# vinayak-gholap1993/Geometric-Multigrid-preconditioners-for-long-range-Coulomb-interaction

Hardware: AMD Instinct MI355X
Metric: DoF/s per CG-iter (GMG-precond Poisson, 3D) (higher is better)
Workload: dtype f64

## Files before the change

### geometric-multigrid-preconditioners-for-long-range-coulomb-interaction_amd/csrc/gmg_coulomb.hip

```cpp
#include "../../include/gmg_coulomb.h"
#include "gmg_device.hpp"
#include "gmg_sgs.hpp"
#include "gmg_sgs_phase.hpp"
#include "gmg_sgs_dep.hpp"
#include "gmg_sgs_reg.hpp"
#ifdef GMG_EXPERIMENTS
#include "gmg_sgs_chain.hpp"
#endif
#include "gmg_lattice.hpp"
#include "gmg_transfer.hpp"
#include <hip/hip_ext.h>

#include <algorithm>
#include <array>
#include <chrono>
#include <cmath>
#include <cstdio>
#include <cstdlib>
#include <cstring>
#include <climits>
#include <map>
#include <string>
#include <thread>
#include <unordered_map>
#include <vector>

#include "gmg_comm.hpp"

using namespace gmg;

namespace {

struct DevCSR {
  int64_t n_rows = 0, n_cols = 0, nnz = 0;
  int32_t *rowptr = nullptr, *col = nullptr;
  double *val = nullptr;
  int32_t *tile_row = nullptr;
  int n_tiles = 0, tiles_per_xcd = 0, grid = 0;
  bool valid = false;
  HaloPlan halo;
  bool sell = false;
  int32_t *slice_ptr = nullptr;
  int32_t *slice_base = nullptr;
  void *sell_vals = nullptr;
  void *sell_cols = nullptr;
  double *sell_dict = nullptr;
  int32_t *sell_spat = nullptr, *sell_pat = nullptr;
// ... 58 lines not shown
  double cheb_lmax = 0.0;
  SgsPlan sgs;
};

}

struct gmg_context {
  int device = 0;
  hipStream_t stream = nullptr;
  int n_levels = 0;
  std::vector<Level> lv;
  DevCSR S;
  double *S_invd = nullptr;
  double *S_tmp = nullptr;
  int smoother = GMG_SMOOTHER_SSOR;
  double omega = 0.5;
  int steps = 2;
  int cheb_degree = 2;
  double cheb_ratio = 30.0, cheb_lmax_user = 0.0;
  double coarse_tol = 1e-10;
  int coarse_maxit = 1000;
  int64_t cg_n = 0;
  double *cg_g = nullptr, *cg_d0 = nullptr, *cg_d1 = nullptr, *cg_h = nullptr;
  double *cg_ring[kXRing] = {};
  int64_t cg_ring_len = 0;
  char *ring_shared[kPeerMaxRanks] = {};
  int64_t ring_stride = 0;
  int64_t peer_meta[kPeerMaxRanks][4 + kPeerMaxRanks] = {};
  unsigned long long peer_tag0 = 1;
  unsigned int *peer_push_cnt = nullptr;
  CGState *st = nullptr;
  CGState *st_host = nullptr;
  CGState st_final{};
  hipEvent_t ev_chunk[2] = {nullptr, nullptr};
  double *part_a = nullptr, *part_b = nullptr;
  double *scal_dev = nullptr;
  double *scal_host = nullptr;
  int *sgs_abort = nullptr;
  int coarse_chunk = 0;
  int sgs_y_slots = 0;
  bool sgs_disable_wave = false, sgs_disable_phase = false, sgs_chain = false, sgs_dep = false, sgs_reg = false, debug_upload = false, sgs_profile = false;
  int sgs_profile_mode = 0;
  int sgs_phase_chunk = 0;
  int sgs_pf_lead_kb = 0;
  bool sgs_phase_nocascade = false;
  bool sgs_phase_nosplit = false;
  int sgs_phase_profile = 0;
  int sgs_groups = 0;
  int sgs_lds_bytes_override = 0;
  bool disable_sell = false, disable_patterns = false, disable_compression = false, disable_sellp = false, disable_rowclass = false, disable_lattice = false;
  int lattice_segments = 0;
  int lattice_max_blocks = 0;
  int sell_grid = 0;
  int sellp_rr = 0;
  double sellp_cost = 4.0;
  int ssor_blocks = 1;
  int ssor_partition = GMG_SSOR_PARTITION_ROWS;
  std::map<int, std::vector<int64_t>> ssor_block_rows;
  int cg_variant = 0;
  int last_coarse_iters = 0;
  int prof_every = 0;
  std::vector<hipEvent_t> ev_a, ev_b;
  std::vector<hipEvent_t> ev_c, ev_d;
  std::vector<hipEvent_t> ev_e, ev_f;
  bool launch_refused = false;
  int ev_used = 0, ev2_used = 0, ev3_used = 0;
  long long sgs_launch_no = 0;
  hipEvent_t timed_start = nullptr, timed_stop = nullptr;
  gmg_stats stats{};
  double *dens_dev = nullptr;
  int64_t dens_cells = 0;
  int dens_nq = 0;
  Comm comm;
  bool dist = false;
  int64_t sys_global = 0, l0_global = 0;
  double *sys_full_a = nullptr, *sys_full_b = nullptr;
  std::string err;
};

namespace {

#define HIPC(call)                                                                                   \
  do {                                                                                               \
    hipError_t e_ = (call);                                                                          \
    if (e_ != hipSuccess) {                                                                          \
      ctx->err = std::string(#call) + ": " + hipGetErrorString(e_);                                  \
      return GMG_ERR_HIP;                                                                            \
    }                                                                                                \
  } while (0)

#define CHK(call)                 \
  do {                            \
// ... 942 lines not shown
        hipLaunchKernelGGL(vec_add_kernel, dim3(g), dim3(kThreads), 0, ctx->stream, u, 1.0, (const double *)y, L.n);
      }
    }
  }
  *u_io = u;
  return launch_status(ctx);
}

void collect_profile_samples(gmg_context *ctx) {
  const int iters = ctx->st_final.iters;
  for (int i = 0; i < ctx->ev_used; ++i) {
    float ms = 0.f;
    if (hipEventElapsedTime(&ms, ctx->ev_a[(size_t)i], ctx->ev_b[(size_t)i]) != hipSuccess) continue;
    if (i * ctx->prof_every < iters) {
      ctx->stats.spmv0_ms_total += ms;
      ctx->stats.spmv0_samples++;
    } else {
      ctx->stats.spmv0_noop_ms_total += ms;
      ctx->stats.spmv0_noop_samples++;
    }
  }
  for (int i = 0; i < ctx->ev2_used; ++i) {
    float ms = 0.f;
    if (hipEventElapsedTime(&ms, ctx->ev_c[(size_t)i], ctx->ev_d[(size_t)i]) != hipSuccess) continue;
    if (i * ctx->prof_every < iters) {
      ctx->stats.cgupd_ms_total += ms;
      ctx->stats.cgupd_samples++;
    }
  }
}

constexpr int64_t kUnfusedMinRowsDecl = 200000;

template <class EnqueueOne>
int run_cg_chunks(gmg_context *ctx, int later_default, EnqueueOne enqueue_one) {
  const int maxit = ctx->coarse_maxit;
  const int last = ctx->last_coarse_iters;
  const int first = ctx->coarse_chunk > 0 ? ctx->coarse_chunk : (last > 8 ? last - (later_default < 6 ? std::max(2, last / 4) : 2) : 16);
  const int later = ctx->coarse_chunk > 0 ? ctx->coarse_chunk : later_default;
  int launched = 0;
  auto launch_chunk = [&](int n, int slot) -> int {
    for (int q = 0; q < n; ++q) {
      const int rc = enqueue_one(launched++);
      if (rc != GMG_OK) return rc;
    }
    CHK(launch_status(ctx));
    HIPC(hipMemcpyAsync(&ctx->st_host[slot], ctx->st, sizeof(CGState), hipMemcpyDeviceToHost, ctx->stream));
    HIPC(hipEventRecord(ctx->ev_chunk[slot], ctx->stream));
    return GMG_OK;
  };
  int slot = 0;
  CHK(launch_chunk(std::min(first, maxit + 1), slot));
  const bool speculate = !l0_partitioned(ctx) || ctx->comm.peer;
  for (;;) {
    if (speculate) CHK(launch_chunk(later, slot ^ 1));
    for (;;) {
      const hipError_t e = hipEventQuery(ctx->ev_chunk[slot]);
      if (e == hipSuccess) break;
      if (e != hipErrorNotReady) { ctx->err = std::string("hipEventQuery: ") + hipGetErrorString(e); return GMG_ERR_HIP; }
    }
    if (ctx->st_host[slot].done) { ctx->st_final = ctx->st_host[slot]; ctx->stats.coarse_enqueued += launched; break; }
    if (launched > maxit + 2 * later + 2) return fail(ctx, GMG_ERR_HIP, "coarse CG state machine did not terminate");
    if (!speculate) CHK(launch_chunk(later, slot ^ 1));
    slot ^= 1;
  }
  return GMG_OK;
}


int coarse_solve_unfused(gmg_context *ctx, double *x, const double *b, int *iters_out, double *res_out);
void collect_profile_samples(gmg_context *ctx);

int coarse_solve(gmg_context *ctx, double *x, const double *b, int *iters_out, double *res_out) {
// ... 954 lines not shown
    tiles.push_back((int32_t)e);
    r = e;
  }
  return tiles;
}

DevCSR *which_matrix(gmg_context *ctx, int which) {
  if (which == GMG_SYSTEM) return &ctx->S;
  if (which < 0 || which >= ctx->n_levels) return nullptr;
  return &ctx->lv[(size_t)which].A;
}

}

#include "gmg_dist.hpp"


extern "C" {

int gmg_create(gmg_context **out, int device_id, int n_levels) {
  if (!out || n_levels < 1) return GMG_ERR_INVALID;
  *out = nullptr;
  int count = 0;
  if (hipGetDeviceCount(&count) != hipSuccess || count <= 0 || device_id < 0 || device_id >= count) return GMG_ERR_HIP;
  if (hipSetDevice(device_id) != hipSuccess) return GMG_ERR_HIP;
  gmg_context *ctx = new gmg_context();
  ctx->device = device_id;
  ctx->n_levels = n_levels;
  ctx->lv.resize((size_t)n_levels);
  auto bail = [&](int code) { gmg_destroy(ctx); return code; };
  if (hipStreamCreateWithFlags(&ctx->stream, hipStreamNonBlocking) != hipSuccess) return bail(GMG_ERR_HIP);
  if (hipMalloc(&ctx->st, sizeof(CGState)) != hipSuccess) return bail(GMG_ERR_HIP);
  if (hipHostMalloc((void **)&ctx->st_host, 2 * sizeof(CGState), hipHostMallocDefault) != hipSuccess) return bail(GMG_ERR_HIP);
  for (auto &e : ctx->ev_chunk)
    if (hipEventCreateWithFlags(&e, hipEventDisableTiming) != hipSuccess) return bail(GMG_ERR_HIP);
  if (hipMalloc(&ctx->part_a, sizeof(double) * 4 * kMaxPartials) != hipSuccess) return bail(GMG_ERR_HIP);
  if (hipMalloc(&ctx->part_b, sizeof(double) * 4 * kMaxPartials) != hipSuccess) return bail(GMG_ERR_HIP);
  if (hipMalloc(&ctx->scal_dev, sizeof(double) * 8) != hipSuccess) return bail(GMG_ERR_HIP);
  if (hipHostMalloc((void **)&ctx->scal_host, sizeof(double) * 8, hipHostMallocDefault) != hipSuccess) return bail(GMG_ERR_HIP);
  if (hipHostMalloc((void **)&ctx->sgs_abort, sizeof(int), hipHostMallocDefault) != hipSuccess) return bail(GMG_ERR_HIP);
  *ctx->sgs_abort = 0;
  (void)hipMemsetAsync(ctx->st, 0, sizeof(CGState), ctx->stream);
  if (const char *env = std::getenv("GMG_OPTIONS")) {
    std::string all(env);
    size_t pos = 0;
    while (pos < all.size()) {
      size_t end = all.find(',', pos);
      if (end == std::string::npos) end = all.size();
      const std::string item = all.substr(pos, end - pos);
      pos = end + 1;
      const size_t eq = item.find('=');
      if (item.empty()) continue;
      const std::string key = eq == std::string::npos ? item : item.substr(0, eq);
      const double v = eq == std::string::npos ? 1.0 : std::atof(item.c_str() + eq + 1);
      if (gmg_set_option(ctx, key.c_str(), v) != GMG_OK) return bail(GMG_ERR_INVALID);
    }
  }
  *out = ctx;
  return GMG_OK;
}

int gmg_destroy(gmg_context *ctx) {
  if (!ctx) return GMG_OK;
  (void)hipSetDevice(ctx->device);
  if (ctx->stream) (void)hipStreamSynchronize(ctx->stream);
  release_operators(ctx);
  if (ctx->peer_push_cnt) (void)hipFree(ctx->peer_push_cnt);
  if (ctx->dens_dev) (void)hipFree(ctx->dens_dev);
  comm_destroy(ctx->comm);
  for (double *p : {ctx->part_a, ctx->part_b, ctx->scal_dev})
    if (p) (void)hipFree(p);
  if (ctx->st) (void)hipFree(ctx->st);
  if (ctx->st_host) (void)hipHostFree(ctx->st_host);
  for (auto &e : ctx->ev_chunk)
    if (e) (void)hipEventDestroy(e);
  if (ctx->scal_host) (void)hipHostFree(ctx->scal_host);
  if (ctx->sgs_abort) (void)hipHostFree(ctx->sgs_abort);
  for (auto *v : {&ctx->ev_a, &ctx->ev_b, &ctx->ev_c, &ctx->ev_d, &ctx->ev_e, &ctx->ev_f})
    for (hipEvent_t e : *v) (void)hipEventDestroy(e);
  if (ctx->stream) (void)hipStreamDestroy(ctx->stream);
  delete ctx;
  return GMG_OK;
}

int gmg_reset(gmg_context *ctx, int n_levels) {
  if (!ctx || n_levels < 1) return GMG_ERR_INVALID;
  (void)hipSetDevice(ctx->device);
  HIPC(hipStreamSynchronize(ctx->stream));
  release_operators(ctx);
  ctx->n_levels = n_levels;
  ctx->lv.assign((size_t)n_levels, Level());
  ctx->last_coarse_iters = 0;
  ctx->stats = gmg_stats{};
  ctx->ev3_used = 0;
  return GMG_OK;
}

const char *gmg_last_error(const gmg_context *ctx) { return ctx ? ctx->err.c_str() : "null context"; }

int gmg_synchronize(gmg_context *ctx) {
  if (!ctx) return GMG_ERR_INVALID;
  HIPC(hipStreamSynchronize(ctx->stream));
  return GMG_OK;
}

int gmg_set_system_matrix(gmg_context *ctx, int64_t n_rows, int64_t n_cols, const int64_t *rowptr, const int32_t *col,
// ... 862 lines not shown
  for (int pass = 0; pass < 2; ++pass) {
    HIPC(hipEventRecord(e0, ctx->stream));
    for (int r = 0; r < reps; ++r)
      hipLaunchKernelGGL(stream_copy_kernel, dim3(kMaxPartials * 2), dim3(kThreads), 0, ctx->stream, (const double2 *)a, b, n2);
    HIPC(hipEventRecord(e1, ctx->stream));
    HIPC(hipEventSynchronize(e1));
    HIPC(hipEventElapsedTime(&ms, e0, e1));
  }
  if (copy_gbps) *copy_gbps = (double)n2 * 32 * reps / (ms * 1e-3) / 1e9;
  (void)hipEventDestroy(e0); (void)hipEventDestroy(e1);
  (void)hipFree(a); (void)hipFree(b);
  return GMG_OK;
}

int gmg_set_option(gmg_context *ctx, const char *key, double value) {
  if (!ctx || !key) return GMG_ERR_INVALID;
  const std::string k(key);
  const bool on = value != 0.0;
  if (k == "host_threads") g_host_threads = (int)value;
  else if (k == "debug_upload") ctx->debug_upload = on;
  else if (k == "disable_sell") ctx->disable_sell = on;
  else if (k == "disable_patterns") ctx->disable_patterns = on;
  else if (k == "disable_compression") ctx->disable_compression = on;
  else if (k == "disable_sellp") ctx->disable_sellp = on;
  else if (k == "disable_rowclass") ctx->disable_rowclass = on;
  else if (k == "disable_lattice") ctx->disable_lattice = on;
  else if (k == "lattice_segments") ctx->lattice_segments = (int)value;
  else if (k == "lattice_max_blocks") ctx->lattice_max_blocks = (int)value;
  else if (k == "sell_grid") ctx->sell_grid = (int)value;
  else if (k == "sellp_cost") ctx->sellp_cost = value;
  else if (k == "sellp_rr") ctx->sellp_rr = (int)value;
  else if (k == "cg_variant") ctx->cg_variant = (int)value;
  else if (k == "coarse_chunk") ctx->coarse_chunk = (int)value;
  else if (k == "ssor_balanced") ctx->ssor_partition = on ? GMG_SSOR_PARTITION_BALANCED : GMG_SSOR_PARTITION_ROWS;
  else if (k == "sgs_y_slots") ctx->sgs_y_slots = (int)value;
  else if (k == "sgs_disable_wave") ctx->sgs_disable_wave = on;
  else if (k == "sgs_disable_phase") ctx->sgs_disable_phase = on;
  else if (k == "sgs_dep") ctx->sgs_dep = on;
  else if (k == "sgs_reg") ctx->sgs_reg = on;
  else if (k == "sgs_pf_lead_kb") ctx->sgs_pf_lead_kb = (int)value;
  else if (k == "sgs_chain") {
#ifndef GMG_EXPERIMENTS
    if (on) return fail(ctx, GMG_ERR_UNSUPPORTED, "sgs_chain needs a -DGMG_EXPERIMENTS build (tools/build_experiments.sh)");
#endif
    ctx->sgs_chain = on;
  }
  else if (k == "sgs_phase_profile") {
    if (on && ctx->dist && ctx->comm.n_ranks > 1) return fail(ctx, GMG_ERR_INVALID, "sgs_phase_profile: one rank only (the instrumented sweep is a single-GPU measurement)");
    ctx->sgs_phase_profile = (int)value;
  }
  else if (k == "sgs_phase_nosplit") ctx->sgs_phase_nosplit = on;
  else if (k == "sgs_phase_nocascade") ctx->sgs_phase_nocascade = on;
  else if (k == "sgs_phase_chunk") ctx->sgs_phase_chunk = (int)value;
  else if (k == "sgs_groups") ctx->sgs_groups = (int)value;
  else if (k == "sgs_lds_bytes_override") ctx->sgs_lds_bytes_override = (int)value;
  else if (k == "sgs_profile") {
    if (on && ctx->dist && ctx->comm.n_ranks > 1) return fail(ctx, GMG_ERR_INVALID, "sgs_profile: one rank only");
    ctx->sgs_profile = on;
    ctx->sgs_profile_mode = (int)value - 1;
#ifndef GMG_EXPERIMENTS
    if (ctx->sgs_profile_mode > 0) return fail(ctx, GMG_ERR_UNSUPPORTED, "sgs_profile modes > 1 need a -DGMG_EXPERIMENTS build (tools/build_experiments.sh)");
#endif
  }
  else return fail(ctx, GMG_ERR_INVALID, "gmg_set_option: unknown key");
  return GMG_OK;
}
// ... 70 lines not shown
```

### geometric-multigrid-preconditioners-for-long-range-coulomb-interaction_amd/csrc/gmg_device.hpp

```cpp
#pragma once
#include <hip/hip_runtime.h>
#include <stdint.h>

#include <type_traits>

namespace gmg {

constexpr int kThreads = 256;
constexpr int kTileNnz = 4096;
constexpr int kPasses = kTileNnz / (kThreads * 4);
constexpr int kMaxPartials = 2048;


__device__ __forceinline__ double wave_sum(double v) {
#pragma unroll
  for (int off = 32; off > 0; off >>= 1) v += __shfl_down(v, off, 64);
  return v;
}

__device__ __forceinline__ double wave_max(double v) {
#pragma unroll
  for (int off = 32; off > 0; off >>= 1) v = fmax(v, __shfl_down(v, off, 64));
  return v;
}

__device__ __forceinline__ double block_sum(double v, double *scratch ) {
  v = wave_sum(v);
  const int lane = threadIdx.x & 63, wid = threadIdx.x >> 6;
  __syncthreads();
  if (lane == 0) scratch[wid] = v;
  __syncthreads();
  return ((scratch[0] + scratch[1]) + scratch[2]) + scratch[3];
}

__device__ __forceinline__ double block_max(double v, double *scratch) {
  v = wave_max(v);
  const int lane = threadIdx.x & 63, wid = threadIdx.x >> 6;
  __syncthreads();
  if (lane == 0) scratch[wid] = v;
  __syncthreads();
  return fmax(fmax(scratch[0], scratch[1]), fmax(scratch[2], scratch[3]));
}

__device__ __forceinline__ double reduce_partials(const double *p, int n, double *scratch) {
  double s = 0.0;
  for (int i = threadIdx.x; i < n; i += kThreads) s += p[i];
  return block_sum(s, scratch);
}


constexpr int kXRing = 8;

struct CGState {
  double gh[2];
  double res0;
  double res;
  int it_k1;
  int it_k2;
  int done;
  int status;
  int iters;
  int pad;
  double alpha[kXRing];
};

constexpr int kPeerRanks = 8;
constexpr int kPeerCgOffset = 4096;
struct PeerCG {
  char *area;
  char *peer_area[kPeerRanks];
  int n_ranks, me;
  unsigned nb_mask;
  unsigned long long tag0;
  int *abort_flag;
};
constexpr long long kPeerCgSpinLimit = 30000000LL;

__device__ __forceinline__ bool peer_cg_wait(const PeerCG &pc, const unsigned long long *tags, unsigned mask, unsigned long long want) {
  __shared__ int ok_s;
  if (threadIdx.x == 0) {
// ... 45 lines not shown
  double *w;
  double omega, c1;
  const double *g;
  double *dnew;
  CGState *st;
  const double *part_in;
  int n_part_in;
  double *part_out;
  double tol;
  int maxit;
};

__device__ __forceinline__ bool cg_open_iteration(CGState *st, const double *part_in, int n_part_in, double tol, int maxit,
                                                  double *red, double *beta_out) {
  if (st->done) return false;
  const double gg = reduce_partials(part_in, n_part_in, red);
  const double res = sqrt(gg);
  const int it = st->it_k2;
  const bool conv = res <= tol;
  const bool fail = !conv && (it >= maxit || res != res);
  const bool writer = blockIdx.x == 0 && threadIdx.x == 0;
  if (conv || fail) {
    if (writer) {
      st->done = 1;
      st->status = conv ? 0 : 1;
      st->res = res;
      st->iters = it;
      if (it == 0) st->res0 = res;
    }
    return false;
  }
  const double gh_new = res * res;
  *beta_out = (it == 0) ? 0.0 : gh_new / st->gh[(it & 1) ^ 1];
  if (writer) {
    st->gh[it & 1] = gh_new;
    st->it_k1 = it;
    if (it == 0) st->res0 = res;
  }
  return true;
}

template <int MODE, int CG>
__global__ __launch_bounds__(kThreads) void spmv_tile_kernel(SpmvArgs a) {
  __shared__ __attribute__((aligned(16))) double prod[kTileNnz + 8];
  __shared__ double red[4];
  const int tid = threadIdx.x;
  constexpr bool XFORM = (CG == 1);

  double beta = 0.0;
  if constexpr (CG == 1) {
    if (!cg_open_iteration(a.st, a.part_in, a.n_part_in, a.tol, a.maxit, red, &beta)) return;
  }
  if constexpr (CG == 2) {
    if (a.st->done) return;
  }

  const int xcd = blockIdx.x & 7, lb = blockIdx.x >> 3, nb = gridDim.x >> 3;
  const int t_begin = xcd * a.tiles_per_xcd;
  const int t_end = min(t_begin + a.tiles_per_xcd, a.n_tiles);
  double dot_acc = 0.0;

  for (int t = t_begin + lb; t < t_end; t += nb) {
    const int r0 = a.tile_row[t], r1 = a.tile_row[t + 1];
    const int k0 = a.rowptr[r0], k1 = a.rowptr[r1];
    const int ka = k0 & ~3;
    if (k1 - ka <= kTileNnz) {
// ... 541 lines not shown
        const uchar4 k0 = kq;
        if (q + 1 < qe) { kq = kbase[(size_t)(q + 1) * 64]; cols_of(q + 1, c); }
        acc += dict[k0.x] * v0; acc += dict[k0.y] * v1; acc += dict[k0.z] * v2; acc += dict[k0.w] * v3;
      }
    }
    if (valid) finish(row, acc, self, have_self);
    ++s;
  }
  if constexpr (CG != 0) {
    const double sblock = block_sum(dot_acc, red);
    if (threadIdx.x == 0) a.part_out[blockIdx.x] = sblock;
  }
}

struct CGDirArgs {
  double *d;
  const double *d_old;
  const double *g;
  int64_t n;
  CGState *st;
  const double *part_in;
  int n_part_in;
  double tol;
  int maxit;
  PeerCG pc;
  int n_nb;
  int nb_rank[kPeerRanks];
  const int32_t *send_idx;
  int send_off[kPeerRanks + 1];
  double *peer_ghost[kPeerRanks];
  long long peer_stride[kPeerRanks];
  unsigned int *cnt;
  int n_push_wg;
};
__global__ __launch_bounds__(kThreads) void cg_direction_kernel(CGDirArgs a) {
  __shared__ double red[4];
  if (a.st->done) return;
  const int64_t n2 = a.n >> 1;
  const double2 *o2 = reinterpret_cast<const double2 *>(a.d_old);
  const double2 *g2 = reinterpret_cast<const double2 *>(a.g);
  double2 *d2 = reinterpret_cast<double2 *>(a.d);
  const int64_t i0 = (int64_t)blockIdx.x * kThreads + threadIdx.x, stride = (int64_t)gridDim.x * kThreads;
  double2 ov{0.0, 0.0}, gv{0.0, 0.0};
  if (i0 < n2) { ov = o2[i0]; gv = g2[i0]; }
  double beta = 0.0;
  const int it = a.st->it_k2;
  if (!cg_open_iteration(a.st, a.part_in, a.n_part_in, a.tol, a.maxit, red, &beta)) return;
  for (int64_t i = i0; i < n2; i += stride) {
    if (i != i0) { ov = o2[i]; gv = g2[i]; }
    double2 dv;
    dv.x = beta * ov.x - gv.x; dv.y = beta * ov.y - gv.y;
    d2[i] = dv;
  }
  if ((a.n & 1) && blockIdx.x == 0 && threadIdx.x == 0) {
    const int64_t i = a.n - 1;
    a.d[i] = beta * a.d_old[i] - a.g[i];
  }
  if (a.pc.area && (int)blockIdx.x < a.n_push_wg) {
    for (int i = 0; i < a.n_nb; ++i) {
      double *dst = a.peer_ghost[i] + (long long)(it & 7) * a.peer_stride[i];
      const int cnt = a.send_off[i + 1] - a.send_off[i];
      for (int k = blockIdx.x * kThreads + threadIdx.x; k < cnt; k += a.n_push_wg * kThreads) {
        const int li = a.send_idx[a.send_off[i] + k];
        dst[k] = beta * a.d_old[li] - a.g[li];
      }
    }
    __threadfence_system();
    __syncthreads();
    if (threadIdx.x == 0 && atomicAdd(a.cnt, 1u) == (unsigned)a.n_push_wg - 1u) {
      *a.cnt = 0;
      for (int i = 0; i < a.n_nb; ++i)
        __hip_atomic_store(reinterpret_cast<unsigned long long *>(a.pc.peer_area[a.nb_rank[i]] + 2048 + (it & 7) * 64) + a.pc.me,
                           a.pc.tag0 + (unsigned long long)it + 1ull, __ATOMIC_RELEASE, __HIP_MEMORY_SCOPE_SYSTEM);
    }
  }
}

struct PeerSumArgs {
  PeerCG pc;
  const double *part;
// ... 84 lines not shown
  if (i0 < n2) { dv = d2[i0]; hv = h2[i0]; xv = x2[i0]; gv = g2[i0]; }
  const double dh = reduce_partials(a.part_dh, a.n_part_dh, red);
  const int it = a.st->it_k1;
  const double alpha = a.st->gh[it & 1] / dh;
  double acc = 0.0;
  for (int64_t i = i0; i < n2; i += stride) {
    if (i != i0) { dv = d2[i]; hv = h2[i]; xv = x2[i]; gv = g2[i]; }
    xv.x += alpha * dv.x; xv.y += alpha * dv.y;
    gv.x += alpha * hv.x; gv.y += alpha * hv.y;
    x2[i] = xv; g2[i] = gv;
    acc += gv.x * gv.x;
    acc += gv.y * gv.y;
  }
  if ((a.n & 1) && blockIdx.x == 0 && threadIdx.x == 0) {
    const int64_t i = a.n - 1;
    a.x[i] += alpha * a.d[i];
    const double gi = a.g[i] + alpha * a.h[i];
    a.g[i] = gi;
    acc += gi * gi;
  }
  const double s = block_sum(acc, red);
  if (threadIdx.x == 0) a.part_gg[blockIdx.x] = s;
  if (blockIdx.x == 0 && threadIdx.x == 0) a.st->it_k2 = it + 1;
}

struct CGUpdateGArgs {
  double *g;
  const double *h;
  int64_t n;
  CGState *st;
  const double *part_dh;
  int n_part_dh;
  double *part_gg;
};
__global__ __launch_bounds__(kThreads) void cg_update_g_kernel(CGUpdateGArgs a) {
  __shared__ double red[4];
  if (a.st->done) return;
  const int64_t n2 = a.n >> 1;
  const double2 *h2 = reinterpret_cast<const double2 *>(a.h);
  double2 *g2 = reinterpret_cast<double2 *>(a.g);
  const int64_t i0 = (int64_t)blockIdx.x * kThreads + threadIdx.x, stride = (int64_t)gridDim.x * kThreads;
  double2 hv{0.0, 0.0}, gv{0.0, 0.0};
  if (i0 < n2) { hv = h2[i0]; gv = g2[i0]; }
  const int it = a.st->it_k1;
  const double dh = reduce_partials(a.part_dh, a.n_part_dh, red);
  const double alpha = a.st->gh[it & 1] / dh;
  double acc = 0.0;
  for (int64_t i = i0; i < n2; i += stride) {
    if (i != i0) { hv = h2[i]; gv = g2[i]; }
    gv.x += alpha * hv.x; gv.y += alpha * hv.y;
    g2[i] = gv;
    acc += gv.x * gv.x;
    acc += gv.y * gv.y;
  }
  if ((a.n & 1) && blockIdx.x == 0 && threadIdx.x == 0) {
    const int64_t i = a.n - 1;
    const double gi = a.g[i] + alpha * a.h[i];
    a.g[i] = gi;
    acc += gi * gi;
  }
  const double s = block_sum(acc, red);
  if (threadIdx.x == 0) a.part_gg[blockIdx.x] = s;
  if (blockIdx.x == 0 && threadIdx.x == 0) {
    a.st->alpha[it % kXRing] = alpha;
    a.st->it_k2 = it + 1;
  }
}

struct CGXFlushArgs {
  double *x;
  const double *ring[kXRing];
  int64_t n;
  const CGState *st;
  int lo, upto;
};
__global__ __launch_bounds__(kThreads) void cg_xflush_kernel(CGXFlushArgs a) {
  const int hi = min(a.st->it_k2, a.upto);
  if (hi <= a.lo) return;
  const int64_t n2 = a.n >> 1;
// ... 295 lines not shown
```

### geometric-multigrid-preconditioners-for-long-range-coulomb-interaction_amd/csrc/gmg_dist.hpp

```cpp
#pragma once

namespace {

constexpr int64_t kUnfusedMinRows = 200000;

int coarse_solve_unfused(gmg_context *ctx, double *x, const double *b, int *iters_out, double *res_out) {
  Level &L0 = ctx->lv[0];
  DevCSR &A = L0.A;
  const bool comm = l0_partitioned(ctx);
  const int64_t n = L0.n;
  const int g_vec = grid_for(n);
  const int g_upd = grid_for(n / 2);
  double *s_gg = ctx->scal_dev + 4, *s_dh = ctx->scal_dev + 5;
  const bool peer = comm && ctx->comm.peer;
  if (!ctx->cg_ring[0]) {
    if (peer) {
      ctx->ring_stride = (A.n_cols + 2 + 15) / 16 * 16;
      if (comm_share_alloc(ctx->comm, sizeof(double) * (size_t)(ctx->ring_stride * kXRing), ctx->ring_shared))
        return fail(ctx, GMG_ERR_COMM, "coarse CG: shared direction vectors could not be mapped");
      for (int r = 0; r < kXRing; ++r) ctx->cg_ring[r] = reinterpret_cast<double *>(ctx->ring_shared[ctx->comm.rank]) + (int64_t)r * ctx->ring_stride;
      int64_t mine[4 + kPeerMaxRanks];
      mine[0] = ctx->ring_stride; mine[1] = n; mine[2] = mine[3] = 0;
      for (int r = 0; r < kPeerMaxRanks; ++r) mine[4 + r] = -1;
      int64_t ro = 0;
      for (int i = 0; i < A.halo.n_neighbors; ++i) { mine[4 + A.halo.rank[(size_t)i]] = ro; ro += A.halo.recv_count[(size_t)i]; }
      if (comm_exchange_meta(ctx->comm, mine, 4 + kPeerMaxRanks, ctx->peer_meta)) return fail(ctx, GMG_ERR_COMM, "coarse CG: meta exchange failed");
      if (!ctx->peer_push_cnt) {
        HIPC(hipMalloc(&ctx->peer_push_cnt, sizeof(unsigned int)));
        HIPC(hipMemsetAsync(ctx->peer_push_cnt, 0, sizeof(unsigned int), ctx->stream));
      }
    } else {
      for (int r = 0; r < kXRing; ++r) CHK(alloc_vec(ctx, &ctx->cg_ring[r], A.n_cols));
    }
    ctx->cg_ring_len = A.n_cols;
  }
  if (ctx->cg_ring_len < A.n_cols) return fail(ctx, GMG_ERR_INVALID, "coarse CG ring sized for a smaller operator");
  PeerCG pc{};
  if (peer) {
    pc.area = ctx->comm.box[ctx->comm.rank] + kPeerCgOffset;
    for (int r = 0; r < ctx->comm.n_ranks; ++r) pc.peer_area[r] = ctx->comm.box[r] + kPeerCgOffset;
    pc.n_ranks = ctx->comm.n_ranks; pc.me = ctx->comm.rank;
    for (int i = 0; i < A.halo.n_neighbors; ++i)
      if (A.halo.recv_count[(size_t)i] > 0) pc.nb_mask |= 1u << A.halo.rank[(size_t)i];
    pc.tag0 = ctx->peer_tag0;
    ctx->peer_tag0 += (unsigned long long)ctx->coarse_maxit + 16ull;
    pc.abort_flag = ctx->comm.abort_host;
  }
  auto peer_sum = [&](const double *part, int n_part, int kind, int from_init, double *out) {
    PeerSumArgs ps{pc, part, n_part, kind, from_init, ctx->st, out};
    hipLaunchKernelGGL(peer_allsum_kernel, dim3(1), dim3(kThreads), 0, ctx->stream, ps);
  };

  CGInitArgs ia{b, x, ctx->cg_g, ctx->cg_ring[kXRing - 1], ctx->cg_ring[kXRing - 1], n, ctx->st, ctx->part_b};
  hipLaunchKernelGGL(cg_init_kernel, dim3(g_vec), dim3(kThreads), 0, ctx->stream, ia);
  const double *gg_src = ctx->part_b;
  int gg_n = g_vec;
  if (peer) {
    peer_sum(ctx->part_b, g_vec, 0, 1, s_gg);
    gg_src = s_gg; gg_n = 1;
  } else if (comm) {
    hipLaunchKernelGGL(reduce_final_kernel, dim3(1), dim3(kThreads), 0, ctx->stream, (const double *)ctx->part_b, g_vec, 1, 0u, s_gg);
    if (allreduce_sum(ctx->comm, s_gg, 1, ctx->stream)) return fail(ctx, GMG_ERR_COMM, "all-reduce failed");
    gg_src = s_gg; gg_n = 1;
  }

  const int maxit = ctx->coarse_maxit;
  ctx->ev_used = 0; ctx->ev2_used = 0;
  auto flush_x = [&](int lo, int upto) {
    CGXFlushArgs fa{};
    fa.x = x; fa.n = n; fa.st = ctx->st; fa.lo = lo; fa.upto = upto;
    for (int r = 0; r < kXRing; ++r) fa.ring[r] = ctx->cg_ring[r];
    hipLaunchKernelGGL(cg_xflush_kernel, dim3(g_upd), dim3(kThreads), 0, ctx->stream, fa);
  };
  int launched_total = 0;
  CHK(run_cg_chunks(ctx, (!comm && L0.n >= kUnfusedMinRows) ? 3 : 6, [&](int launched) -> int {
    launched_total = launched + 1;
    double *d = ctx->cg_ring[launched % kXRing];
    CGDirArgs da{};
    da.d = d; da.d_old = ctx->cg_ring[(launched + kXRing - 1) % kXRing]; da.g = ctx->cg_g; da.n = n; da.st = ctx->st;
    da.part_in = gg_src; da.n_part_in = gg_n; da.tol = ctx->coarse_tol; da.maxit = maxit;
    if (peer) {
      da.pc = pc;
      da.send_idx = A.halo.send_idx; da.cnt = ctx->peer_push_cnt;
      int so = 0;
      for (int i = 0; i < A.halo.n_neighbors; ++i) {
        if (A.halo.send_count[(size_t)i] > 0) {
          const int k = da.n_nb++, pr = A.halo.rank[(size_t)i];
          da.nb_rank[k] = pr; da.send_off[k] = so; da.send_off[k + 1] = so + A.halo.send_count[(size_t)i];
          da.peer_stride[k] = ctx->peer_meta[pr][0];
          da.peer_ghost[k] = reinterpret_cast<double *>(ctx->ring_shared[pr]) + ctx->peer_meta[pr][1] + ctx->peer_meta[pr][4 + ctx->comm.rank];
          if (ctx->peer_meta[pr][4 + ctx->comm.rank] < 0) return fail(ctx, GMG_ERR_INVALID, "coarse CG: the neighbours' halo plans disagree");
        }
        so += A.halo.send_count[(size_t)i];
      }
      da.n_push_wg = da.n_nb ? std::min(g_vec, 16) : 0;
    }
    hipLaunchKernelGGL(cg_direction_kernel, dim3(g_vec), dim3(kThreads), 0, ctx->stream, da);
    if (comm && !peer && halo_exchange(ctx->comm, A.halo, d, n, ctx->stream)) return fail(ctx, GMG_ERR_COMM, "halo exchange failed");
    if (peer && pc.nb_mask) hipLaunchKernelGGL(peer_wait_halo_kernel, dim3(1), dim3(64), 0, ctx->stream, pc, (const CGState *)ctx->st);
    SpmvArgs a = base_args(A, d, ctx->cg_h);
    a.st = ctx->st;
    a.part_out = ctx->part_a;
    const bool sample = ctx->prof_every > 0 && (launched % ctx->prof_every) == 0 && ctx->ev_used < (int)ctx->ev_a.size();
    if (sample) { ctx->timed_start = ctx->ev_a[(size_t)ctx->ev_used]; ctx->timed_stop = ctx->ev_b[(size_t)ctx->ev_used++]; }
    const int n_part_dh = launch_op<kStore, 2>(ctx, A, a);
    const double *dh_src = ctx->part_a;
    int dh_n = n_part_dh;
    if (peer) {
      peer_sum(ctx->part_a, n_part_dh, 1, 0, s_dh);
      dh_src = s_dh; dh_n = 1;
    } else if (comm) {
      hipLaunchKernelGGL(reduce_final_kernel, dim3(1), dim3(kThreads), 0, ctx->stream, (const double *)ctx->part_a, n_part_dh, 1, 0u, s_dh);
      if (allreduce_sum(ctx->comm, s_dh, 1, ctx->stream)) return fail(ctx, GMG_ERR_COMM, "all-reduce failed");
      dh_src = s_dh; dh_n = 1;
    }
    CGUpdateGArgs ua{ctx->cg_g, ctx->cg_h, n, ctx->st, dh_src, dh_n, ctx->part_b};
    const bool sample2 = sample && ctx->ev2_used < (int)ctx->ev_c.size();
    if (sample2) { ctx->timed_start = ctx->ev_c[(size_t)ctx->ev2_used]; ctx->timed_stop = ctx->ev_d[(size_t)ctx->ev2_used++]; }
    launch_timed(ctx, cg_update_g_kernel, dim3(g_upd), dim3(kThreads), 0, ua);
    if ((launched + 1) % kXRing == 0) flush_x(launched + 1 - kXRing, launched + 1);
    if (peer) {
      peer_sum(ctx->part_b, g_upd, 0, 0, s_gg);
    } else if (comm) {
      hipLaunchKernelGGL(reduce_final_kernel, dim3(1), dim3(kThreads), 0, ctx->stream, (const double *)ctx->part_b, g_upd, 1, 0u, s_gg);
      if (allreduce_sum(ctx->comm, s_gg, 1, ctx->stream)) return fail(ctx, GMG_ERR_COMM, "all-reduce failed");
    } else {
      gg_src = ctx->part_b; gg_n = g_upd;
    }
    return GMG_OK;
  }));
  flush_x(launched_total / kXRing * kXRing, INT_MAX);
  collect_profile_samples(ctx);
  ctx->last_coarse_iters = ctx->st_final.iters;
  ctx->stats.coarse_solves++;
  ctx->stats.coarse_iterations += ctx->st_final.iters;
  if (iters_out) *iters_out = ctx->st_final.iters;
  if (res_out) *res_out = ctx->st_final.res;
  if (ctx->st_final.status != 0) {
    if (comm_aborted(ctx->comm)) return fail(ctx, GMG_ERR_COMM, "coarse CG: a rank gave up waiting for its neighbours' sums or halo entries");
    ctx->err = "coarse CG did not converge within max_it (stopped at iteration " + std::to_string(ctx->st_final.iters) + ", residual " + std::to_string(ctx->st_final.res) + ")";
    return GMG_ERR_COARSE_NOCONV;
  }
  return GMG_OK;
}

}
```

Baseline: 145.2 million.

## Drive coarse CG with host-polled mapped progress word instead of chunked event sync

Adds a fast coarse-CG path for single-rank runs. The device publishes iteration progress and final status to coherent mapped host memory, and the host polls it to enqueue only a few iterations ahead, replacing chunked speculative launches plus event and memcpy sync. The direction and update kernels get a FAST template that issues the state, partials and vector loads together before a single block reduction, and drops the early done check. This aims to cut over-enqueued no-op launches and host sync latency, at the cost of busy host polling and system-scope atomics in the kernels.

```diff
diff --git a/geometric-multigrid-preconditioners-for-long-range-coulomb-interaction_amd/csrc/gmg_coulomb.hip b/geometric-multigrid-preconditioners-for-long-range-coulomb-interaction_amd/csrc/gmg_coulomb.hip
--- a/geometric-multigrid-preconditioners-for-long-range-coulomb-interaction_amd/csrc/gmg_coulomb.hip
+++ b/geometric-multigrid-preconditioners-for-long-range-coulomb-interaction_amd/csrc/gmg_coulomb.hip
@@ -13,6 +13,7 @@
 
 #include <algorithm>
 #include <array>
+#include <atomic>
 #include <chrono>
 #include <cmath>
 #include <cstdio>
@@ -137,6 +138,8 @@
   CGState *st = nullptr;
   CGState *st_host = nullptr;
   CGState st_final{};
+  CGState *st_pub = nullptr;
+  CGState *st_pub_dev = nullptr;
   hipEvent_t ev_chunk[2] = {nullptr, nullptr};
   double *part_a = nullptr, *part_b = nullptr;
   double *scal_dev = nullptr;
@@ -163,6 +166,7 @@
   int ssor_partition = GMG_SSOR_PARTITION_ROWS;
   std::map<int, std::vector<int64_t>> ssor_block_rows;
   int cg_variant = 0;
+  bool coarse_fast = true;
   int last_coarse_iters = 0;
   int prof_every = 0;
   std::vector<hipEvent_t> ev_a, ev_b;
@@ -1171,13 +1175,51 @@
 
 constexpr int64_t kUnfusedMinRowsDecl = 200000;
 
+constexpr double kCoarsePollLimitS = 60.0;
+
 template <class EnqueueOne>
-int run_cg_chunks(gmg_context *ctx, int later_default, EnqueueOne enqueue_one) {
+int run_cg_chunks(gmg_context *ctx, int later_default, EnqueueOne enqueue_one, bool publish = false) {
   const int maxit = ctx->coarse_maxit;
   const int last = ctx->last_coarse_iters;
+  int launched = 0;
+  if (publish) {
+    const int ahead = ctx->coarse_chunk > 0 ? ctx->coarse_chunk : later_default;
+    const int first = std::min(last > 8 ? last - std::max(2, last / 4) : 16, maxit + 1);
+    volatile CGState *pub = ctx->st_pub;
+    pub->it_k2 = 0; pub->done = 0;
+    std::atomic_thread_fence(std::memory_order_seq_cst);
+    auto enqueue = [&](int n) -> int {
+      for (int q = 0; q < n; ++q) {
+        const int rc = enqueue_one(launched++);
+        if (rc != GMG_OK) return rc;
+      }
+      return launch_status(ctx);
+    };
+    CHK(enqueue(first));
+    int seen = -1;
+    auto t_seen = std::chrono::steady_clock::now();
+    for (unsigned polls = 0;; ++polls) {
+      if (pub->done) {
+        std::atomic_thread_fence(std::memory_order_acquire);
+        ctx->st_final = CGState{};
+        ctx->st_final.done = 1; ctx->st_final.status = pub->status; ctx->st_final.iters = pub->iters; ctx->st_final.res = pub->res;
+        ctx->stats.coarse_enqueued += launched;
+        break;
+      }
+      const int started = pub->it_k2;
+      if (started != seen) {
+        seen = started;
+        t_seen = std::chrono::steady_clock::now();
+      } else if ((polls & 1023u) == 1023u &&
+                 std::chrono::duration<double>(std::chrono::steady_clock::now() - t_seen).count() > kCoarsePollLimitS) {
+        return fail(ctx, GMG_ERR_HIP, "coarse CG: no progress of the device iteration for 60 s");
+      }
+      if (launched <= maxit && launched < started + ahead) CHK(enqueue(1));
+    }
+    return GMG_OK;
+  }
   const int first = ctx->coarse_chunk > 0 ? ctx->coarse_chunk : (last > 8 ? last - (later_default < 6 ? std::max(2, last / 4) : 2) : 16);
   const int later = ctx->coarse_chunk > 0 ? ctx->coarse_chunk : later_default;
-  int launched = 0;
   auto launch_chunk = [&](int n, int slot) -> int {
     for (int q = 0; q < n; ++q) {
       const int rc = enqueue_one(launched++);
@@ -2198,6 +2240,9 @@
   if (hipStreamCreateWithFlags(&ctx->stream, hipStreamNonBlocking) != hipSuccess) return bail(GMG_ERR_HIP);
   if (hipMalloc(&ctx->st, sizeof(CGState)) != hipSuccess) return bail(GMG_ERR_HIP);
   if (hipHostMalloc((void **)&ctx->st_host, 2 * sizeof(CGState), hipHostMallocDefault) != hipSuccess) return bail(GMG_ERR_HIP);
+  if (hipHostMalloc((void **)&ctx->st_pub, sizeof(CGState), hipHostMallocCoherent | hipHostMallocMapped) != hipSuccess) return bail(GMG_ERR_HIP);
+  std::memset(ctx->st_pub, 0, sizeof(CGState));
+  if (hipHostGetDevicePointer((void **)&ctx->st_pub_dev, ctx->st_pub, 0) != hipSuccess) return bail(GMG_ERR_HIP);
   for (auto &e : ctx->ev_chunk)
     if (hipEventCreateWithFlags(&e, hipEventDisableTiming) != hipSuccess) return bail(GMG_ERR_HIP);
   if (hipMalloc(&ctx->part_a, sizeof(double) * 4 * kMaxPartials) != hipSuccess) return bail(GMG_ERR_HIP);
@@ -2238,6 +2283,7 @@
     if (p) (void)hipFree(p);
   if (ctx->st) (void)hipFree(ctx->st);
   if (ctx->st_host) (void)hipHostFree(ctx->st_host);
+  if (ctx->st_pub) (void)hipHostFree(ctx->st_pub);
   for (auto &e : ctx->ev_chunk)
     if (e) (void)hipEventDestroy(e);
   if (ctx->scal_host) (void)hipHostFree(ctx->scal_host);
@@ -3166,6 +3212,7 @@
   else if (k == "sellp_rr") ctx->sellp_rr = (int)value;
   else if (k == "cg_variant") ctx->cg_variant = (int)value;
   else if (k == "coarse_chunk") ctx->coarse_chunk = (int)value;
+  else if (k == "coarse_fast") ctx->coarse_fast = on;
   else if (k == "ssor_balanced") ctx->ssor_partition = on ? GMG_SSOR_PARTITION_BALANCED : GMG_SSOR_PARTITION_ROWS;
   else if (k == "sgs_y_slots") ctx->sgs_y_slots = (int)value;
   else if (k == "sgs_disable_wave") ctx->sgs_disable_wave = on;
diff --git a/geometric-multigrid-preconditioners-for-long-range-coulomb-interaction_amd/csrc/gmg_device.hpp b/geometric-multigrid-preconditioners-for-long-range-coulomb-interaction_amd/csrc/gmg_device.hpp
--- a/geometric-multigrid-preconditioners-for-long-range-coulomb-interaction_amd/csrc/gmg_device.hpp
+++ b/geometric-multigrid-preconditioners-for-long-range-coulomb-interaction_amd/csrc/gmg_device.hpp
@@ -46,6 +46,21 @@
   double s = 0.0;
   for (int i = threadIdx.x; i < n; i += kThreads) s += p[i];
   return block_sum(s, scratch);
+}
+
+__device__ __forceinline__ double partials_share(const double *p, int n) {
+  constexpr int kPer = kMaxPartials / kThreads;
+  double v[kPer];
+#pragma unroll
+  for (int k = 0; k < kPer; ++k) {
+    const int i = threadIdx.x + k * kThreads;
+    v[k] = i < n ? p[i] : 0.0;
+  }
+  double s = 0.0;
+#pragma unroll
+  for (int k = 0; k < kPer; ++k)
+    if ((int)threadIdx.x + k * kThreads < n) s += v[k];
+  return s;
 }
 
 
@@ -157,6 +172,56 @@
   }
   const double gh_new = res * res;
   *beta_out = (it == 0) ? 0.0 : gh_new / st->gh[(it & 1) ^ 1];
+  if (writer) {
+    st->gh[it & 1] = gh_new;
+    st->it_k1 = it;
+    if (it == 0) st->res0 = res;
+  }
+  return true;
+}
+
+struct CGWords {
+  int done, it_k1, it_k2;
+  double gh0, gh1;
+};
+__device__ __forceinline__ CGWords cg_words(const CGState *st) {
+  CGWords w;
+  w.done = st->done; w.it_k1 = st->it_k1; w.it_k2 = st->it_k2;
+  w.gh0 = st->gh[0]; w.gh1 = st->gh[1];
+  return w;
+}
+#define CG_LANDED(...) asm volatile("" ::__VA_ARGS__)
+
+__device__ __forceinline__ void cg_publish_progress(CGState *pub, int it_started) {
+  __hip_atomic_store(&pub->it_k2, it_started, __ATOMIC_RELAXED, __HIP_MEMORY_SCOPE_SYSTEM);
+}
+__device__ __forceinline__ void cg_publish_final(CGState *pub, double res, int iters, int status) {
+  __hip_atomic_store(&pub->res, res, __ATOMIC_RELAXED, __HIP_MEMORY_SCOPE_SYSTEM);
+  __hip_atomic_store(&pub->iters, iters, __ATOMIC_RELAXED, __HIP_MEMORY_SCOPE_SYSTEM);
+  __hip_atomic_store(&pub->status, status, __ATOMIC_RELAXED, __HIP_MEMORY_SCOPE_SYSTEM);
+  __hip_atomic_store(&pub->done, 1, __ATOMIC_RELEASE, __HIP_MEMORY_SCOPE_SYSTEM);
+}
+
+__device__ __forceinline__ bool cg_open_loaded(CGState *st, CGState *pub, const CGWords &w, double gg, double tol, int maxit,
+                                               double *beta_out) {
+  const double res = sqrt(gg);
+  const int it = w.it_k2;
+  const bool conv = res <= tol;
+  const bool fail = !conv && (it >= maxit || res != res);
+  const bool writer = blockIdx.x == 0 && threadIdx.x == 0;
+  if (conv || fail) {
+    if (writer) {
+      st->done = 1;
+      st->status = conv ? 0 : 1;
+      st->res = res;
+      st->iters = it;
+      if (it == 0) st->res0 = res;
+      if (pub) cg_publish_final(pub, res, it, conv ? 0 : 1);
+    }
+    return false;
+  }
+  const double gh_new = res * res;
+  *beta_out = (it == 0) ? 0.0 : gh_new / ((it & 1) ? w.gh0 : w.gh1);
   if (writer) {
     st->gh[it & 1] = gh_new;
     st->it_k1 = it;
@@ -764,10 +829,14 @@
   long long peer_stride[kPeerRanks];
   unsigned int *cnt;
   int n_push_wg;
-};
+  CGState *pub;
+};
+template <bool FAST>
 __global__ __launch_bounds__(kThreads) void cg_direction_kernel(CGDirArgs a) {
   __shared__ double red[4];
-  if (a.st->done) return;
+  if constexpr (!FAST) {
+    if (a.st->done) return;
+  }
   const int64_t n2 = a.n >> 1;
   const double2 *o2 = reinterpret_cast<const double2 *>(a.d_old);
   const double2 *g2 = reinterpret_cast<const double2 *>(a.g);
@@ -776,8 +845,18 @@
   double2 ov{0.0, 0.0}, gv{0.0, 0.0};
   if (i0 < n2) { ov = o2[i0]; gv = g2[i0]; }
   double beta = 0.0;
-  const int it = a.st->it_k2;
-  if (!cg_open_iteration(a.st, a.part_in, a.n_part_in, a.tol, a.maxit, red, &beta)) return;
+  int it;
+  if constexpr (FAST) {
+    const CGWords w = cg_words(a.st);
+    const double s = partials_share(a.part_in, a.n_part_in);
+    CG_LANDED("v"(ov.x), "v"(ov.y), "v"(gv.x), "v"(gv.y), "v"(s), "v"(w.done), "v"(w.it_k2), "v"(w.gh0), "v"(w.gh1));
+    if (w.done) return;
+    it = w.it_k2;
+    if (!cg_open_loaded(a.st, a.pub, w, block_sum(s, red), a.tol, a.maxit, &beta)) return;
+  } else {
+    it = a.st->it_k2;
+    if (!cg_open_iteration(a.st, a.part_in, a.n_part_in, a.tol, a.maxit, red, &beta)) return;
+  }
   for (int64_t i = i0; i < n2; i += stride) {
     if (i != i0) { ov = o2[i]; gv = g2[i]; }
     double2 dv;
@@ -928,19 +1007,36 @@
   const double *part_dh;
   int n_part_dh;
   double *part_gg;
-};
+  CGState *pub;
+};
+template <bool FAST>
 __global__ __launch_bounds__(kThreads) void cg_update_g_kernel(CGUpdateGArgs a) {
   __shared__ double red[4];
-  if (a.st->done) return;
+  if constexpr (!FAST) {
+    if (a.st->done) return;
+  }
   const int64_t n2 = a.n >> 1;
   const double2 *h2 = reinterpret_cast<const double2 *>(a.h);
   double2 *g2 = reinterpret_cast<double2 *>(a.g);
   const int64_t i0 = (int64_t)blockIdx.x * kThreads + threadIdx.x, stride = (int64_t)gridDim.x * kThreads;
   double2 hv{0.0, 0.0}, gv{0.0, 0.0};
   if (i0 < n2) { hv = h2[i0]; gv = g2[i0]; }
-  const int it = a.st->it_k1;
-  const double dh = reduce_partials(a.part_dh, a.n_part_dh, red);
-  const double alpha = a.st->gh[it & 1] / dh;
+  int it;
+  double alpha;
+  if constexpr (FAST) {
+    const CGWords w = cg_words(a.st);
+    const double s = partials_share(a.part_dh, a.n_part_dh);
+    CG_LANDED("v"(hv.x), "v"(hv.y), "v"(gv.x), "v"(gv.y), "v"(s), "v"(w.done), "v"(w.it_k1), "v"(w.gh0), "v"(w.gh1));
+    if (w.done) return;
+    it = w.it_k1;
+    if (a.pub && blockIdx.x == 0 && threadIdx.x == 0) cg_publish_progress(a.pub, it + 1);
+    const double dh = block_sum(s, red);
+    alpha = ((it & 1) ? w.gh1 : w.gh0) / dh;
+  } else {
+    it = a.st->it_k1;
+    const double dh = reduce_partials(a.part_dh, a.n_part_dh, red);
+    alpha = a.st->gh[it & 1] / dh;
+  }
   double acc = 0.0;
   for (int64_t i = i0; i < n2; i += stride) {
     if (i != i0) { hv = h2[i]; gv = g2[i]; }
diff --git a/geometric-multigrid-preconditioners-for-long-range-coulomb-interaction_amd/csrc/gmg_dist.hpp b/geometric-multigrid-preconditioners-for-long-range-coulomb-interaction_amd/csrc/gmg_dist.hpp
--- a/geometric-multigrid-preconditioners-for-long-range-coulomb-interaction_amd/csrc/gmg_dist.hpp
+++ b/geometric-multigrid-preconditioners-for-long-range-coulomb-interaction_amd/csrc/gmg_dist.hpp
@@ -13,6 +13,7 @@
   const int g_upd = grid_for(n / 2);
   double *s_gg = ctx->scal_dev + 4, *s_dh = ctx->scal_dev + 5;
   const bool peer = comm && ctx->comm.peer;
+  const bool fast = !comm && ctx->coarse_fast;
   if (!ctx->cg_ring[0]) {
     if (peer) {
       ctx->ring_stride = (A.n_cols + 2 + 15) / 16 * 16;
@@ -73,12 +74,14 @@
     hipLaunchKernelGGL(cg_xflush_kernel, dim3(g_upd), dim3(kThreads), 0, ctx->stream, fa);
   };
   int launched_total = 0;
-  CHK(run_cg_chunks(ctx, (!comm && L0.n >= kUnfusedMinRows) ? 3 : 6, [&](int launched) -> int {
+  const int later = fast ? (L0.n >= kUnfusedMinRows ? 2 : 3) : (!comm && L0.n >= kUnfusedMinRows) ? 3 : 6;
+  const int rc_loop = run_cg_chunks(ctx, later, [&](int launched) -> int {
     launched_total = launched + 1;
     double *d = ctx->cg_ring[launched % kXRing];
     CGDirArgs da{};
     da.d = d; da.d_old = ctx->cg_ring[(launched + kXRing - 1) % kXRing]; da.g = ctx->cg_g; da.n = n; da.st = ctx->st;
     da.part_in = gg_src; da.n_part_in = gg_n; da.tol = ctx->coarse_tol; da.maxit = maxit;
+    if (fast) da.pub = ctx->st_pub_dev;
     if (peer) {
       da.pc = pc;
       da.send_idx = A.halo.send_idx; da.cnt = ctx->peer_push_cnt;
@@ -95,7 +98,8 @@
       }
       da.n_push_wg = da.n_nb ? std::min(g_vec, 16) : 0;
     }
-    hipLaunchKernelGGL(cg_direction_kernel, dim3(g_vec), dim3(kThreads), 0, ctx->stream, da);
+    if (fast) hipLaunchKernelGGL(cg_direction_kernel<true>, dim3(g_vec), dim3(kThreads), 0, ctx->stream, da);
+    else hipLaunchKernelGGL(cg_direction_kernel<false>, dim3(g_vec), dim3(kThreads), 0, ctx->stream, da);
     if (comm && !peer && halo_exchange(ctx->comm, A.halo, d, n, ctx->stream)) return fail(ctx, GMG_ERR_COMM, "halo exchange failed");
     if (peer && pc.nb_mask) hipLaunchKernelGGL(peer_wait_halo_kernel, dim3(1), dim3(64), 0, ctx->stream, pc, (const CGState *)ctx->st);
     SpmvArgs a = base_args(A, d, ctx->cg_h);
@@ -114,10 +118,12 @@
       if (allreduce_sum(ctx->comm, s_dh, 1, ctx->stream)) return fail(ctx, GMG_ERR_COMM, "all-reduce failed");
       dh_src = s_dh; dh_n = 1;
     }
-    CGUpdateGArgs ua{ctx->cg_g, ctx->cg_h, n, ctx->st, dh_src, dh_n, ctx->part_b};
+    CGUpdateGArgs ua{ctx->cg_g, ctx->cg_h, n, ctx->st, dh_src, dh_n, ctx->part_b, fast ? ctx->st_pub_dev : nullptr};
+    if (fast && (dh_n > kMaxPartials || gg_n > kMaxPartials)) return fail(ctx, GMG_ERR_INVALID, "coarse CG: more reduction partials than kMaxPartials");
     const bool sample2 = sample && ctx->ev2_used < (int)ctx->ev_c.size();
     if (sample2) { ctx->timed_start = ctx->ev_c[(size_t)ctx->ev2_used]; ctx->timed_stop = ctx->ev_d[(size_t)ctx->ev2_used++]; }
-    launch_timed(ctx, cg_update_g_kernel, dim3(g_upd), dim3(kThreads), 0, ua);
+    if (fast) launch_timed(ctx, cg_update_g_kernel<true>, dim3(g_upd), dim3(kThreads), 0, ua);
+    else launch_timed(ctx, cg_update_g_kernel<false>, dim3(g_upd), dim3(kThreads), 0, ua);
     if ((launched + 1) % kXRing == 0) flush_x(launched + 1 - kXRing, launched + 1);
     if (peer) {
       peer_sum(ctx->part_b, g_upd, 0, 0, s_gg);
@@ -128,7 +134,8 @@
       gg_src = ctx->part_b; gg_n = g_upd;
     }
     return GMG_OK;
-  }));
+  }, fast);
+  CHK(rc_loop);
   flush_x(launched_total / kXRing * kXRing, INT_MAX);
   collect_profile_samples(ctx);
   ctx->last_coarse_iters = ctx->st_final.iters;
```

Measured after the change: 146.5 million, median of 6. About the same (+0.9%).
